# kvcache-ai/ktransformers

Measured on NVIDIA H100. Metric: decode tok/s DeepSeek-V3 671B INT4 (Q4_K_M) MoE-block hot path; HBM GB/s vs roofline, higher is better.
Workload: dtype int8xint4/int6->int32 dp4a, fp32 scales+accumulate, bf16 in/out

## Files before the change

### ktransformers_b200/csrc/elementwise.cu

```cuda
#include <cuda_bf16.h>

#include "common.cuh"

namespace ktb {

__device__ __forceinline__ float block_sum(float v, float* red) {
    v = warp_sum(v);
    const int lane = threadIdx.x & 31, warp = threadIdx.x >> 5, nw = blockDim.x >> 5;
    if (lane == 0) red[warp] = v;
    __syncthreads();
    float s = lane < nw ? red[lane] : 0.f;
    s = warp_sum(s);
    __syncthreads();
    return s;
}
__device__ __forceinline__ float bf(const __nv_bfloat16 v) { return __bfloat162float(v); }

constexpr int kNormThreads = 1024, kNormPairs = 4;
__global__ void __launch_bounds__(kNormThreads) add_rmsnorm_kernel(__nv_bfloat16* resid, const __nv_bfloat16* delta, const __nv_bfloat16* weight, float eps,
                                                                   __nv_bfloat16* out, int H, long resid_stride, long delta_stride, long out_stride) {
    __shared__ float red[32];
    griddep_launch_dependents();
    __nv_bfloat162 wv[kNormPairs];
#pragma unroll
    for (int j = 0; j < kNormPairs; j++) {
        const int i = (threadIdx.x + j * kNormThreads) * 2;
        if (i < H) wv[j] = *reinterpret_cast<const __nv_bfloat162*>(weight + i);
    }
    griddep_wait();
    const long t = blockIdx.x;
    __nv_bfloat16* r = resid + t * resid_stride;
    const __nv_bfloat16* d = delta ? delta + t * delta_stride : nullptr;
    __nv_bfloat162 v[kNormPairs];
    float ss = 0.f;
#pragma unroll
    for (int j = 0; j < kNormPairs; j++) {
        const int i = (threadIdx.x + j * kNormThreads) * 2;
        if (i < H) {
            v[j] = *reinterpret_cast<const __nv_bfloat162*>(r + i);
            if (d) {
                v[j] = __hadd2(v[j], *reinterpret_cast<const __nv_bfloat162*>(d + i));
                *reinterpret_cast<__nv_bfloat162*>(r + i) = v[j];
            }
            const float2 f = __bfloat1622float2(v[j]);
            ss += f.x * f.x + f.y * f.y;
        }
    }
    const float inv = rsqrtf(block_sum(ss, red) / (float)H + eps);
    __nv_bfloat16* o = out + t * out_stride;
#pragma unroll
    for (int j = 0; j < kNormPairs; j++) {
        const int i = (threadIdx.x + j * kNormThreads) * 2;
        if (i < H) {
            const float2 f = __bfloat1622float2(v[j]);
            *reinterpret_cast<__nv_bfloat162*>(o + i) = __hmul2(wv[j], __floats2bfloat162_rn(f.x * inv, f.y * inv));
        }
    }
}

__global__ void __launch_bounds__(256) mla_prep_kernel(const __nv_bfloat16* q, int num_heads, int q_head_dim, int nope_dim, const __nv_bfloat16* kva,
                                                       const __nv_bfloat16* kv_norm_w, float eps, const float* cos_t, const float* sin_t,
                                                       __nv_bfloat16* kv_cache, int page_size, const int* page_idx, const int* page_off,
                                                       __nv_bfloat16* q_pe_out) {
    constexpr int R = 64, LAT = 512;
    __shared__ float red[8];
    griddep_launch_dependents();
    griddep_wait();
    const long t = blockIdx.x;
    const float* cs = cos_t + t * R;
    const float* sn = sin_t + t * R;
    auto rope = [&](const __nv_bfloat16* x, int i) -> float {
        const int half = R / 2;
        const float a = bf(x[i < half ? 2 * i : 2 * (i - half) + 1]);
        const float b = i < half ? -bf(x[2 * i + 1]) : bf(x[2 * (i - half)]);
        const float p0 = __bfloat162float(__float2bfloat16_rn(a * cs[i])), p1 = __bfloat162float(__float2bfloat16_rn(b * sn[i]));
        return p0 + p1;
    };
    for (int u = threadIdx.x; u < num_heads * R; u += blockDim.x) {
        const int h = u / R, i = u - h * R;
        q_pe_out[(t * num_heads + h) * R + i] = __float2bfloat16_rn(rope(q + (t * num_heads + h) * q_head_dim + nope_dim, i));
    }
    __nv_bfloat16* dst = kv_cache + ((long)page_idx[t] * page_size + page_off[t]) * (LAT + R);
    const __nv_bfloat16* row = kva + t * (LAT + R);
    float ss = 0.f;
    for (int i = threadIdx.x; i < LAT; i += blockDim.x) { const float f = bf(row[i]); ss += f * f; }
    const float inv = rsqrtf(block_sum(ss, red) / (float)LAT + eps);
    for (int i = threadIdx.x; i < LAT; i += blockDim.x) {
        const __nv_bfloat16 hn = __float2bfloat16_rn(bf(row[i]) * inv);
        dst[i] = __hmul(kv_norm_w[i], hn);
    }
    if (threadIdx.x < R) dst[LAT + threadIdx.x] = __float2bfloat16_rn(rope(row + LAT, threadIdx.x));
}

}

using namespace ktb;

static bool misaligned(const void* p, uintptr_t bytes) { return ((uintptr_t)p & (bytes - 1)) != 0; }

extern "C" int ktb200_add_rmsnorm(void* residual, const void* delta, const void* weight, float eps, void* out, int n_tokens, int hidden, void* stream) {
    if (!residual || !weight || !out || n_tokens < 0) { set_error("add_rmsnorm: null pointer / negative n_tokens"); return KTB200_EINVAL; }
    if (hidden <= 0 || hidden % 2 || hidden > 2 * kNormPairs * kNormThreads) { set_error("add_rmsnorm: hidden %d must be even and <= 8192 (bf16)", hidden); return KTB200_EINVAL; }
    if (misaligned(residual, 4)) { set_error("add_rmsnorm: residual must be 4-byte aligned"); return KTB200_EINVAL; }
    if (misaligned(delta, 4)) { set_error("add_rmsnorm: delta must be 4-byte aligned"); return KTB200_EINVAL; }
    if (misaligned(weight, 4)) { set_error("add_rmsnorm: weight must be 4-byte aligned"); return KTB200_EINVAL; }
    if (misaligned(out, 4)) { set_error("add_rmsnorm: out must be 4-byte aligned"); return KTB200_EINVAL; }
    if (n_tokens == 0) return KTB200_OK;
    KTB_CUDA_CHECK(launch_pdl(add_rmsnorm_kernel, dim3(n_tokens), dim3(kNormThreads), 0, (cudaStream_t)stream, (__nv_bfloat16*)residual, (const __nv_bfloat16*)delta,
                              (const __nv_bfloat16*)weight, eps, (__nv_bfloat16*)out, hidden, (long)hidden, (long)hidden, (long)hidden));
    count_launch();
    return KTB200_OK;
}

extern "C" int ktb200_mla_prep(const void* q, int num_heads, int qk_nope_head_dim, const void* kv_a_out, const void* kv_a_norm_weight, float eps,
                               const float* cos, const float* sin, void* kv_cache, int page_size, const int* page_idx, const int* page_offset,
                               void* q_pe_out, int n_tokens, void* stream) {
    if (!q || !kv_a_out || !kv_a_norm_weight || !cos || !sin || !kv_cache || !page_idx || !page_offset || !q_pe_out || num_heads <= 0 || qk_nope_head_dim <= 0) {
        set_error("mla_prep: null pointer / bad shape");
        return KTB200_EINVAL;
    }
    if (n_tokens <= 0) return KTB200_OK;
    KTB_CUDA_CHECK(launch_pdl(mla_prep_kernel, dim3(n_tokens), dim3(256), 0, (cudaStream_t)stream, (const __nv_bfloat16*)q, num_heads, qk_nope_head_dim + 64,
                              qk_nope_head_dim, (const __nv_bfloat16*)kv_a_out, (const __nv_bfloat16*)kv_a_norm_weight, eps, cos, sin, (__nv_bfloat16*)kv_cache,
                              page_size, page_idx, page_offset, (__nv_bfloat16*)q_pe_out));
    count_launch();
    return KTB200_OK;
}

namespace ktb {

constexpr int kMaxGridZ = 65535;

__global__ void __launch_bounds__(256) absorb_q_kernel(const __nv_bfloat16* q, long q_head_stride, long q_tok_stride, const __nv_bfloat16* W, int D, int Cc,
                                                        __nv_bfloat16* out) {
    __shared__ float qs[512];
    __shared__ float part[4][512];
    griddep_launch_dependents();
    griddep_wait();
    const int h = blockIdx.y, t = blockIdx.z, heads = gridDim.y;
    const __nv_bfloat16* qrow = q + t * q_tok_stride + h * q_head_stride;
    for (int i = threadIdx.x; i < D; i += blockDim.x) qs[i] = bf(qrow[i]);
    __syncthreads();
    const int grp = threadIdx.x >> 6, ct = threadIdx.x & 63;
    const int c = blockIdx.x * 512 + ct * 8;
    float a[8] = {0.f, 0.f, 0.f, 0.f, 0.f, 0.f, 0.f, 0.f};
    if (c < Cc) {
        const int dper = (D + 3) / 4, d0 = grp * dper, d1 = min(D, d0 + dper);
        const __nv_bfloat16* w = W + ((long)h * D) * Cc + c;
#pragma unroll 8
        for (int d = d0; d < d1; d++) {
            const uint4 raw = *reinterpret_cast<const uint4*>(w + (long)d * Cc);
            const __nv_bfloat162* w2 = reinterpret_cast<const __nv_bfloat162*>(&raw);
            const float qd = qs[d];
#pragma unroll
            for (int i = 0; i < 4; i++) {
                const float2 f = __bfloat1622float2(w2[i]);
                a[2 * i] = fmaf(qd, f.x, a[2 * i]);
                a[2 * i + 1] = fmaf(qd, f.y, a[2 * i + 1]);
            }
        }
    }
#pragma unroll
    for (int i = 0; i < 8; i++) part[grp][ct * 8 + i] = a[i];
    __syncthreads();
    const int cc = threadIdx.x * 2;
    if (blockIdx.x * 512 + cc < Cc) {
        const float s0 = (part[0][cc] + part[1][cc]) + (part[2][cc] + part[3][cc]);
        const float s1 = (part[0][cc + 1] + part[1][cc + 1]) + (part[2][cc + 1] + part[3][cc + 1]);
        *reinterpret_cast<__nv_bfloat162*>(out + ((long)t * heads + h) * Cc + blockIdx.x * 512 + cc) = __floats2bfloat162_rn(s0, s1);
    }
}

__global__ void __launch_bounds__(256) absorb_o_kernel(const __nv_bfloat16* lat, const __nv_bfloat16* W, int V, int Cc, __nv_bfloat16* out) {
    griddep_launch_dependents();
    griddep_wait();
    const int h = blockIdx.y, t = blockIdx.z, heads = gridDim.y, lane = threadIdx.x & 31;
    const int v = blockIdx.x * 8 + (threadIdx.x >> 5);
    if (v >= V) return;
    const __nv_bfloat16* x = lat + ((long)t * heads + h) * Cc;
    const __nv_bfloat16* w = W + ((long)h * V + v) * Cc;
    float acc = 0.f;
    for (int c = lane * 8; c < Cc; c += 256) {
        const uint4 wv = *reinterpret_cast<const uint4*>(w + c), xv = *reinterpret_cast<const uint4*>(x + c);
        const __nv_bfloat162* w2 = reinterpret_cast<const __nv_bfloat162*>(&wv);
        const __nv_bfloat162* x2 = reinterpret_cast<const __nv_bfloat162*>(&xv);
#pragma unroll
        for (int i = 0; i < 4; i++) {
            const float2 a = __bfloat1622float2(w2[i]), b = __bfloat1622float2(x2[i]);
            acc = fmaf(a.x, b.x, acc);
            acc = fmaf(a.y, b.y, acc);
        }
    }
    acc = warp_sum(acc);
    if (lane == 0) out[((long)t * heads + h) * V + v] = __float2bfloat16_rn(acc);
}

}

extern "C" int ktb200_mla_absorb_q(const void* q, long q_head_stride, long q_token_stride, const void* w_uk, int num_heads, int nope_dim, int kv_lora_rank,
                                   void* q_abs_out, int n_tokens, void* stream) {
    if (!q || !w_uk || !q_abs_out || num_heads <= 0) { set_error("mla_absorb_q: null pointer / bad num_heads"); return KTB200_EINVAL; }
    if (nope_dim <= 0 || nope_dim > 512) { set_error("mla_absorb_q: qk_nope_head_dim %d must be in 1..512", nope_dim); return KTB200_EINVAL; }
    if (kv_lora_rank <= 0 || kv_lora_rank % 8) { set_error("mla_absorb_q: kv_lora_rank %d must be a positive multiple of 8", kv_lora_rank); return KTB200_EINVAL; }
    if (misaligned(w_uk, 16)) { set_error("mla_absorb_q: w_uk must be 16-byte aligned"); return KTB200_EINVAL; }
    if (misaligned(q_abs_out, 4)) { set_error("mla_absorb_q: q_abs_out must be 4-byte aligned"); return KTB200_EINVAL; }
    if (n_tokens <= 0) return KTB200_OK;
    for (int t0 = 0; t0 < n_tokens; t0 += kMaxGridZ) {
        const int nt = n_tokens - t0 < kMaxGridZ ? n_tokens - t0 : kMaxGridZ;
        KTB_CUDA_CHECK(launch_pdl(ktb::absorb_q_kernel, dim3((kv_lora_rank + 511) / 512, num_heads, nt), dim3(256), 0, (cudaStream_t)stream,
                                  (const __nv_bfloat16*)q + t0 * q_token_stride, q_head_stride, q_token_stride, (const __nv_bfloat16*)w_uk, nope_dim,
                                  kv_lora_rank, (__nv_bfloat16*)q_abs_out + (long)t0 * num_heads * kv_lora_rank));
        count_launch();
    }
    return KTB200_OK;
}

extern "C" int ktb200_mla_absorb_o(const void* attn_latent, const void* w_uv, int num_heads, int v_head_dim, int kv_lora_rank, void* out, int n_tokens, void* stream) {
    if (!attn_latent || !w_uv || !out || num_heads <= 0 || v_head_dim <= 0) { set_error("mla_absorb_o: null pointer / bad shape"); return KTB200_EINVAL; }
    if (kv_lora_rank <= 0 || kv_lora_rank % 8) { set_error("mla_absorb_o: kv_lora_rank %d must be a positive multiple of 8", kv_lora_rank); return KTB200_EINVAL; }
    if (misaligned(attn_latent, 16)) { set_error("mla_absorb_o: attn_latent must be 16-byte aligned"); return KTB200_EINVAL; }
    if (misaligned(w_uv, 16)) { set_error("mla_absorb_o: w_uv must be 16-byte aligned"); return KTB200_EINVAL; }
    if (n_tokens <= 0) return KTB200_OK;
    for (int t0 = 0; t0 < n_tokens; t0 += kMaxGridZ) {
        const int nt = n_tokens - t0 < kMaxGridZ ? n_tokens - t0 : kMaxGridZ;
        KTB_CUDA_CHECK(launch_pdl(ktb::absorb_o_kernel, dim3((v_head_dim + 7) / 8, num_heads, nt), dim3(256), 0, (cudaStream_t)stream,
                                  (const __nv_bfloat16*)attn_latent + (long)t0 * num_heads * kv_lora_rank, (const __nv_bfloat16*)w_uv, v_head_dim,
                                  kv_lora_rank, (__nv_bfloat16*)out + (long)t0 * num_heads * v_head_dim));
        count_launch();
    }
    return KTB200_OK;
}
```

Before: 160.3.

## Parallelize MLA prep across head chunks and prefetch absorb weights before PDL wait

mla_prep now launches a second grid dimension so the q_pe RoPE work for all heads is spread over extra blocks, and the last block handles the KV-cache norm and RoPE. absorb_q and absorb_o issue L2 bulk prefetches of their weight slabs before griddep_wait, so weight loading overlaps the tail of the previous kernel. absorb_o also computes four output rows per warp, reusing each loaded activation vector and using fewer blocks. A profiling script for the attention layer is added. The changes add more blocks and extra prefetch traffic in exchange for lower latency in the attention path.

```diff
diff --git a/ktransformers_b200/csrc/elementwise.cu b/ktransformers_b200/csrc/elementwise.cu
--- a/ktransformers_b200/csrc/elementwise.cu
+++ b/ktransformers_b200/csrc/elementwise.cu
@@ -58,10 +58,11 @@
     }
 }
 
-__global__ void __launch_bounds__(256) mla_prep_kernel(const __nv_bfloat16* q, int num_heads, int q_head_dim, int nope_dim, const __nv_bfloat16* kva,
-                                                       const __nv_bfloat16* kv_norm_w, float eps, const float* cos_t, const float* sin_t,
-                                                       __nv_bfloat16* kv_cache, int page_size, const int* page_idx, const int* page_off,
-                                                       __nv_bfloat16* q_pe_out) {
+constexpr int kPrepThreads = 256;
+__global__ void __launch_bounds__(kPrepThreads) mla_prep_kernel(const __nv_bfloat16* q, int num_heads, int q_head_dim, int nope_dim, const __nv_bfloat16* kva,
+                                                                const __nv_bfloat16* kv_norm_w, float eps, const float* cos_t, const float* sin_t,
+                                                                __nv_bfloat16* kv_cache, int page_size, const int* page_idx, const int* page_off,
+                                                                __nv_bfloat16* q_pe_out) {
     constexpr int R = 64, LAT = 512;
     __shared__ float red[8];
     griddep_launch_dependents();
@@ -76,9 +77,13 @@
         const float p0 = __bfloat162float(__float2bfloat16_rn(a * cs[i])), p1 = __bfloat162float(__float2bfloat16_rn(b * sn[i]));
         return p0 + p1;
     };
-    for (int u = threadIdx.x; u < num_heads * R; u += blockDim.x) {
-        const int h = u / R, i = u - h * R;
-        q_pe_out[(t * num_heads + h) * R + i] = __float2bfloat16_rn(rope(q + (t * num_heads + h) * q_head_dim + nope_dim, i));
+    if (blockIdx.y + 1 < gridDim.y) {
+        const int u = blockIdx.y * kPrepThreads + threadIdx.x;
+        if (u < num_heads * R) {
+            const int h = u / R, i = u - h * R;
+            q_pe_out[(t * num_heads + h) * R + i] = __float2bfloat16_rn(rope(q + (t * num_heads + h) * q_head_dim + nope_dim, i));
+        }
+        return;
     }
     __nv_bfloat16* dst = kv_cache + ((long)page_idx[t] * page_size + page_off[t]) * (LAT + R);
     const __nv_bfloat16* row = kva + t * (LAT + R);
@@ -120,7 +125,9 @@
         return KTB200_EINVAL;
     }
     if (n_tokens <= 0) return KTB200_OK;
-    KTB_CUDA_CHECK(launch_pdl(mla_prep_kernel, dim3(n_tokens), dim3(256), 0, (cudaStream_t)stream, (const __nv_bfloat16*)q, num_heads, qk_nope_head_dim + 64,
+    if ((long)num_heads * 64 > 65534L * kPrepThreads) { set_error("mla_prep: num_heads %d too large", num_heads); return KTB200_EINVAL; }
+    const int chunks = (num_heads * 64 + kPrepThreads - 1) / kPrepThreads;
+    KTB_CUDA_CHECK(launch_pdl(mla_prep_kernel, dim3(n_tokens, chunks + 1), dim3(kPrepThreads), 0, (cudaStream_t)stream, (const __nv_bfloat16*)q, num_heads, qk_nope_head_dim + 64,
                               qk_nope_head_dim, (const __nv_bfloat16*)kv_a_out, (const __nv_bfloat16*)kv_a_norm_weight, eps, cos, sin, (__nv_bfloat16*)kv_cache,
                               page_size, page_idx, page_offset, (__nv_bfloat16*)q_pe_out));
     count_launch();
@@ -136,8 +143,13 @@
     __shared__ float qs[512];
     __shared__ float part[4][512];
     griddep_launch_dependents();
-    griddep_wait();
     const int h = blockIdx.y, t = blockIdx.z, heads = gridDim.y;
+    if (t == 0) {
+        const int c0 = blockIdx.x * 512;
+        const __nv_bfloat16* slab = W + (long)h * D * Cc + c0;
+        for (int d = threadIdx.x; d < D; d += blockDim.x) prefetch_l2_bulk(slab + (long)d * Cc, (uint32_t)min(512, Cc - c0) * 2);
+    }
+    griddep_wait();
     const __nv_bfloat16* qrow = q + t * q_tok_stride + h * q_head_stride;
     for (int i = threadIdx.x; i < D; i += blockDim.x) qs[i] = bf(qrow[i]);
     __syncthreads();
@@ -171,28 +183,40 @@
     }
 }
 
+constexpr int kAbsorbORows = 4;
 __global__ void __launch_bounds__(256) absorb_o_kernel(const __nv_bfloat16* lat, const __nv_bfloat16* W, int V, int Cc, __nv_bfloat16* out) {
     griddep_launch_dependents();
-    griddep_wait();
     const int h = blockIdx.y, t = blockIdx.z, heads = gridDim.y, lane = threadIdx.x & 31;
-    const int v = blockIdx.x * 8 + (threadIdx.x >> 5);
-    if (v >= V) return;
+    const int v0 = blockIdx.x * 8 * kAbsorbORows + (threadIdx.x >> 5) * kAbsorbORows, nv = min(kAbsorbORows, V - v0);
+    if (nv <= 0) return;
+    const __nv_bfloat16* w = W + ((long)h * V + v0) * Cc;
+    if (t == 0 && lane == 0) prefetch_l2_bulk(w, (uint32_t)(nv * Cc) * 2);
+    griddep_wait();
     const __nv_bfloat16* x = lat + ((long)t * heads + h) * Cc;
-    const __nv_bfloat16* w = W + ((long)h * V + v) * Cc;
-    float acc = 0.f;
+    float acc[kAbsorbORows] = {0.f, 0.f, 0.f, 0.f};
     for (int c = lane * 8; c < Cc; c += 256) {
-        const uint4 wv = *reinterpret_cast<const uint4*>(w + c), xv = *reinterpret_cast<const uint4*>(x + c);
-        const __nv_bfloat162* w2 = reinterpret_cast<const __nv_bfloat162*>(&wv);
+        const uint4 xv = *reinterpret_cast<const uint4*>(x + c);
         const __nv_bfloat162* x2 = reinterpret_cast<const __nv_bfloat162*>(&xv);
-#pragma unroll
-        for (int i = 0; i < 4; i++) {
-            const float2 a = __bfloat1622float2(w2[i]), b = __bfloat1622float2(x2[i]);
-            acc = fmaf(a.x, b.x, acc);
-            acc = fmaf(a.y, b.y, acc);
-        }
-    }
-    acc = warp_sum(acc);
-    if (lane == 0) out[((long)t * heads + h) * V + v] = __float2bfloat16_rn(acc);
+        uint4 wv[kAbsorbORows];
+#pragma unroll
+        for (int r = 0; r < kAbsorbORows; r++)
+            wv[r] = r < nv ? *reinterpret_cast<const uint4*>(w + (long)r * Cc + c) : make_uint4(0, 0, 0, 0);
+#pragma unroll
+        for (int r = 0; r < kAbsorbORows; r++) {
+            const __nv_bfloat162* w2 = reinterpret_cast<const __nv_bfloat162*>(&wv[r]);
+#pragma unroll
+            for (int i = 0; i < 4; i++) {
+                const float2 a = __bfloat1622float2(w2[i]), b = __bfloat1622float2(x2[i]);
+                acc[r] = fmaf(a.x, b.x, acc[r]);
+                acc[r] = fmaf(a.y, b.y, acc[r]);
+            }
+        }
+    }
+#pragma unroll
+    for (int r = 0; r < kAbsorbORows; r++) {
+        const float s = warp_sum(acc[r]);
+        if (lane == 0 && r < nv) out[((long)t * heads + h) * V + v0 + r] = __float2bfloat16_rn(s);
+    }
 }
 
 }
@@ -223,7 +247,7 @@
     if (n_tokens <= 0) return KTB200_OK;
     for (int t0 = 0; t0 < n_tokens; t0 += kMaxGridZ) {
         const int nt = n_tokens - t0 < kMaxGridZ ? n_tokens - t0 : kMaxGridZ;
-        KTB_CUDA_CHECK(launch_pdl(ktb::absorb_o_kernel, dim3((v_head_dim + 7) / 8, num_heads, nt), dim3(256), 0, (cudaStream_t)stream,
+        KTB_CUDA_CHECK(launch_pdl(ktb::absorb_o_kernel, dim3((v_head_dim + 8 * kAbsorbORows - 1) / (8 * kAbsorbORows), num_heads, nt), dim3(256), 0, (cudaStream_t)stream,
                                   (const __nv_bfloat16*)attn_latent + (long)t0 * num_heads * kv_lora_rank, (const __nv_bfloat16*)w_uv, v_head_dim,
                                   kv_lora_rank, (__nv_bfloat16*)out + (long)t0 * num_heads * v_head_dim));
         count_launch();
diff --git a/profiles/attn_layer_probe.py b/profiles/attn_layer_probe.py
--- /dev/null
+++ b/profiles/attn_layer_probe.py
@@ -0,0 +1,162 @@
+import argparse
+import ctypes as C
+import os
+import subprocess
+import sys
+
+import torch
+
+ROOT = os.path.dirname(os.path.dirname(os.path.abspath(__file__)))
+sys.path.insert(0, ROOT)
+from ktransformers_b200 import native
+from ktransformers_b200.util.synth import synth_blocks
+
+Q4_K, BF16 = 12, 30
+NL, H, NH, QL, KVL, ROPE, NOPE, VD, PAGE = 61, 7168, 128, 1536, 512, 64, 128, 128, 64
+
+
+def card():
+    try:
+        q = subprocess.run(["nvidia-smi", "--query-gpu=name,power.limit,clocks.max.sm", "--format=csv,noheader", "-i", "0"],
+                           capture_output=True, text=True, timeout=30).stdout.strip()
+    except (OSError, subprocess.SubprocessError):
+        q = ""
+    return q or torch.cuda.get_device_name(0) + " (power limit and clock: nvidia-smi unavailable)"
+
+
+def main():
+    ap = argparse.ArgumentParser()
+    ap.add_argument("--ctx", type=int, default=4096)
+    ap.add_argument("--reps", type=int, default=5, help="timed windows of 10 graph replays; the median is printed")
+    args = ap.parse_args()
+    assert torch.cuda.is_available(), "this probe measures on the GPU"
+    lib = native.lib()
+    dev = "cuda"
+    S = lambda: torch.cuda.current_stream().cuda_stream
+    bf = torch.bfloat16
+    g = torch.Generator(device=dev); g.manual_seed(4242)
+    ctx = args.ctx
+
+    def linear(inf, outf, seed):
+        w = synth_blocks(Q4_K, outf * inf, dev, seed)
+        h = C.c_void_p()
+        native.check(lib.ktb200_linear_create(inf, outf, w.data_ptr(), Q4_K, BF16, 8, 0, C.byref(h)))
+        native.check(lib.ktb200_linear_load_weights(h, S()))
+        return h, w
+
+    def normw(n):
+        return (1.0 + 0.1 * torch.randn(n, device=dev, generator=g)).to(bf)
+
+    pages = (ctx + PAGE) // PAGE + 1
+    att = []
+    for l in range(NL):
+        att.append(dict(qkv_a=linear(H, QL + KVL + ROPE, 9000 + 10 * l), q_b=linear(QL, NH * (NOPE + ROPE), 9002 + 10 * l),
+                        o=linear(NH * VD, H, 9003 + 10 * l),
+                        w_uk=(torch.randn(NH, NOPE, KVL, device=dev, generator=g) * 0.05).to(bf),
+                        w_uv=(torch.randn(NH, VD, KVL, device=dev, generator=g) * 0.05).to(bf),
+                        ln_in=normw(H), ln_qa=normw(QL), ln_kv=normw(KVL), ln_post=normw(H),
+                        cache=(torch.randn(pages, PAGE, KVL + ROPE, device=dev, generator=g) * 0.5).to(bf)))
+    x = (torch.randn(1, H, device=dev, generator=g) * 0.5).to(bf); hbuf = torch.zeros(1, H, dtype=bf, device=dev)
+    y = (torch.randn(1, H, device=dev, generator=g) * 0.02).to(bf)
+    qkva = torch.zeros(1, QL + KVL + ROPE, dtype=bf, device=dev)
+    qa, kva = qkva[:, :QL], qkva[:, QL:]
+    qan = torch.zeros(1, QL, dtype=bf, device=dev)
+    q = torch.zeros(1, NH * (NOPE + ROPE), dtype=bf, device=dev); q_pe = torch.zeros(NH, ROPE, dtype=bf, device=dev)
+    q_abs = torch.zeros(NH, 1, KVL, dtype=bf, device=dev); lat = torch.zeros(1, NH, KVL, dtype=bf, device=dev)
+    o_in = torch.zeros(NH, 1, VD, dtype=bf, device=dev); attn_out = torch.zeros(1, H, dtype=bf, device=dev)
+    inv = 1.0 / (10000.0 ** (torch.arange(0, ROPE, 2, device=dev).float() / ROPE))
+    ang = torch.cat([inv * ctx, inv * ctx])[None]
+    cos, sin = ang.cos().contiguous(), ang.sin().contiguous()
+    pidx = torch.tensor([ctx // PAGE], dtype=torch.int32, device=dev); poff = torch.tensor([ctx % PAGE], dtype=torch.int32, device=dev)
+    ptab = torch.arange(pages, dtype=torch.int32, device=dev)[None].contiguous()
+    klen = torch.tensor([ctx + 1], dtype=torch.int32, device=dev)
+    wsb = lib.ktb200_mla_workspace_bytes(1, NH, 0)
+    ws = torch.zeros(wsb, dtype=torch.uint8, device=dev)
+    mla = [native.MlaParams(1, NH, PAGE, pages, 0, float((NOPE + ROPE) ** -0.5), q_abs.data_ptr(), q_pe.data_ptr(), a["cache"].data_ptr(),
+                            ptab.data_ptr(), klen.data_ptr(), lat.data_ptr(), None, ws.data_ptr(), wsb, pages * PAGE) for a in att]
+    eps = 1e-6
+
+    def lin(hd, src, dst):
+        native.check(lib.ktb200_linear_forward(hd[0], 1, src.data_ptr(), dst.data_ptr(), None, None, S()))
+
+    def q4k(inf, outf):
+        return outf * inf * 144 // 256
+
+    ops = [
+        ("add_rmsnorm 7168 (input)", 5 * H * 2,
+         lambda l: native.check(lib.ktb200_add_rmsnorm(x.data_ptr(), y.data_ptr(), att[l]["ln_in"].data_ptr(), eps, hbuf.data_ptr(), 1, H, S()))),
+        ("qkv_a 7168->2112 Q4_K", q4k(H, QL + KVL + ROPE), lambda l: lin(att[l]["qkv_a"], hbuf, qkva)),
+        ("rmsnorm 1536 (q_a)", 3 * QL * 2,
+         lambda l: native.check(lib.ktb200_add_rmsnorm(qa.data_ptr(), None, att[l]["ln_qa"].data_ptr(), eps, qan.data_ptr(), 1, QL, S()))),
+        ("q_b 1536->24576 Q4_K", q4k(QL, NH * (NOPE + ROPE)), lambda l: lin(att[l]["q_b"], qan, q)),
+        ("mla_prep (128 heads, page 64)", (2 * NH * ROPE + 3 * (KVL + ROPE)) * 2,
+         lambda l: native.check(lib.ktb200_mla_prep(q.data_ptr(), NH, NOPE, kva.data_ptr(), att[l]["ln_kv"].data_ptr(), eps, cos.data_ptr(),
+                                                    sin.data_ptr(), att[l]["cache"].data_ptr(), PAGE, pidx.data_ptr(), poff.data_ptr(),
+                                                    q_pe.data_ptr(), 1, S()))),
+        ("absorb_q (W_UK)", NH * NOPE * KVL * 2,
+         lambda l: native.check(lib.ktb200_mla_absorb_q(q.data_ptr(), NOPE + ROPE, NH * (NOPE + ROPE), att[l]["w_uk"].data_ptr(), NH, NOPE, KVL,
+                                                        q_abs.data_ptr(), 1, S()))),
+        (f"mla_decode ctx {ctx}", (ctx + 1) * (KVL + ROPE) * 2, lambda l: native.check(lib.ktb200_mla_decode(C.byref(mla[l]), S()))),
+        ("absorb_o (W_UV)", NH * VD * KVL * 2,
+         lambda l: native.check(lib.ktb200_mla_absorb_o(lat.data_ptr(), att[l]["w_uv"].data_ptr(), NH, VD, KVL, o_in.data_ptr(), 1, S()))),
+        ("o_proj 16384->7168 Q4_K", q4k(NH * VD, H), lambda l: lin(att[l]["o"], o_in.view(1, NH * VD), attn_out)),
+        ("add_rmsnorm 7168 (post)", 5 * H * 2,
+         lambda l: native.check(lib.ktb200_add_rmsnorm(x.data_ptr(), attn_out.data_ptr(), att[l]["ln_post"].data_ptr(), eps, hbuf.data_ptr(), 1, H, S()))),
+    ]
+
+    def capture(fn):
+        fn(); torch.cuda.synchronize()
+        side = torch.cuda.Stream(); side.wait_stream(torch.cuda.current_stream())
+        with torch.cuda.stream(side):
+            fn()
+        torch.cuda.current_stream().wait_stream(side); torch.cuda.synchronize()
+        gr = torch.cuda.CUDAGraph()
+        with torch.cuda.graph(gr):
+            fn()
+        for _ in range(3):
+            gr.replay()
+        torch.cuda.synchronize()
+        return gr
+
+    def per_layer_us(fn):
+        gr = capture(fn)
+        e0, e1 = torch.cuda.Event(enable_timing=True), torch.cuda.Event(enable_timing=True)
+        t = []
+        for _ in range(args.reps):
+            e0.record()
+            for _ in range(10):
+                gr.replay()
+            e1.record(); torch.cuda.synchronize()
+            t.append(e0.elapsed_time(e1) / 10 / NL * 1e3)
+        return sorted(t)[len(t) // 2]
+
+    print(f"card: {card()}", flush=True)
+    print(f"ctx {ctx}, batch 1; each op 61x with distinct weights in one CUDA graph; median of {args.reps} windows of 10 replays", flush=True)
+    print(f"{'op':34s} {'us/layer':>9s} {'bytes':>12s} {'GB/s':>7s}")
+    total_us, total_b = 0.0, 0
+    for name, nbytes, fn in ops:
+        us = per_layer_us(lambda: [fn(l) for l in range(NL)])
+        total_us += us; total_b += nbytes
+        print(f"{name:34s} {us:9.2f} {nbytes:12d} {nbytes / us / 1e3:7.0f}", flush=True)
+
+    from torch.profiler import ProfilerActivity, profile
+    dec = [o for o in ops if o[0].startswith("mla_decode")][0][2]
+    gr = capture(lambda: [dec(l) for l in range(NL)])
+    with profile(activities=[ProfilerActivity.CUDA]) as prof:
+        gr.replay(); torch.cuda.synchronize()
+    kern = {}
+    for ev in prof.events():
+        if ev.device_type == torch.autograd.DeviceType.CUDA and "mla" in ev.name:
+            kern[ev.name] = kern.get(ev.name, 0.0) + ev.device_time
+    for name, t in sorted(kern.items()):
+        print(f"    of which {name[:60]}: {t / NL:.2f} us (profiler duration)", flush=True)
+
+    chain_us = per_layer_us(lambda: [fn(l) for l in range(NL) for _, _, fn in ops])
+    print(f"{'sum of the ops':34s} {total_us:9.2f} {total_b:12d} {total_b / total_us / 1e3:7.0f}")
+    print(f"{'chain (10 launches x 61 layers)':34s} {chain_us:9.2f} {total_b:12d} {total_b / chain_us / 1e3:7.0f}")
+    print(f"chain - sum: {chain_us - total_us:+.2f} us per layer, {(chain_us - total_us) * NL / 1e3:+.3f} ms per token; "
+          f"chain x 61 = {chain_us * NL / 1e3:.3f} ms", flush=True)
+
+
+if __name__ == "__main__":
+    main()
```

After: 160.3 (median of 6 runs). No clear change (-0.1%).
